# jolars/sgdnet

Measured on AMD Instinct MI355X. Metric: saga_epochs_per_sec, higher is better.
Workload: dtype f64

## Files before the change

sgdnet_amd/csrc/batched_geometry.hpp:

```cpp
#pragma once

#include <hip/hip_ext.h>

#include <type_traits>

#include "common.hpp"

#ifndef SGDNET_BIN_BLOCK
#define SGDNET_BIN_BLOCK 1024
#endif
#ifndef SGDNET_BIN_W
#define SGDNET_BIN_W 8
#endif
#ifndef SGDNET_RANGE_BLOCK
#define SGDNET_RANGE_BLOCK 512
#endif
#ifndef SGDNET_LDS_BLOCK
#define SGDNET_LDS_BLOCK 1024
#endif

namespace sgdnet {

constexpr int kGroup = 16;
constexpr int kBlock = 256;

constexpr int kD0Slots = 256;

constexpr int kCStride = 128;
constexpr uint32_t kIdMask = 0x1fffffffu;
constexpr int kInReg8 = 16;

constexpr int kLdsBlock = SGDNET_LDS_BLOCK;
constexpr int kDenseBlock = 256;
constexpr int kDenseVsBlock = 1024;
constexpr int kTileF = 64;

constexpr int kSlabElems = 32;
constexpr int kSlabGroups = kBlock / kSlabElems;

constexpr int kSyncLine = 32;
constexpr int kSyncGo = 0, kSyncExit = 1, kSyncStart = 2, kSyncCnt1 = 3, kSyncCnt2 = kSyncCnt1 + 8,
              kSyncXcd = kSyncCnt2 + 8;
constexpr int kFusedMaxBps = 128;
constexpr int kSyncLines = kSyncXcd + 8;
constexpr int kSyncSticky = kSyncLines;
constexpr int kSyncSeq = kSyncLines + 1;
constexpr int kFusedChunks = 3;
constexpr long long kFusedStartTicks = 2000000;
constexpr long long kFusedWaitTicks = 200000000;

struct __attribute__((aligned(16))) BinEntry {
  uint32_t t;
  uint32_t j;
  double x;
};
static_assert(sizeof(BinEntry) == 16, "bin entries are 16 bytes");

constexpr int kBinBlock = SGDNET_BIN_BLOCK;
constexpr int kBinDraws = kBinBlock / 2;
constexpr int kBinEntCap = 7 * kBinBlock;
constexpr int kBinW = SGDNET_BIN_W;
constexpr int kRangeBlock = SGDNET_RANGE_BLOCK;
constexpr size_t kRangeLdsBytes = 64 * 1024;

constexpr size_t kLdsPerCu = 160 * 1024;
constexpr size_t kLdsStaticReserve = 2 * 1024;
constexpr size_t kLdsTableMax = 80 * 1024;
constexpr int kLdsCap = 96 * 1024;
constexpr int kLdsAll = (int)(kLdsPerCu - kLdsStaticReserve);

template <typename F>
static int with_class_width(int kw, F&& f) {
  if (kw == 1) return f(std::integral_constant<int, 1>{});
  if (kw == 4) return f(std::integral_constant<int, 4>{});
  return f(std::integral_constant<int, 16>{});
}

static inline unsigned clamped_grid(int64_t work, int64_t per_block, int64_t most) {
  const int64_t grid = (work + per_block - 1) / per_block;
  return (unsigned)(grid < 1 ? 1 : grid > most ? most : grid);
// ... 31 lines not shown
```

sgdnet_amd/csrc/batched_plan.cpp:

```cpp
#include <mutex>
#include <set>
#include <utility>

#include "batched_geometry.hpp"
#include "r_rng_bodies.hpp"

namespace sgdnet {

int batched_max_classes() { return 64; }

int lds_target_grid(const SagaDev& d) {
  static const int forced = exp_env_int("SGDNET_LDS_GRID", 0);
  if (forced > 0) return forced;
  const int cus = d.cu_budget > 0 && d.cu_budget < 256 ? d.cu_budget : 256;
  const int g = cus - d.cu_reserve;
  return g < 64 ? 64 : g;
}

size_t binned_max_range_features(int K) { return kRangeLdsBytes / (sizeof(double) * (size_t)K); }

static size_t table_bytes(const SagaDev& d) { return sizeof(double) * (size_t)d.K * (size_t)d.p; }

int allow_dynamic_lds(const void* kernel, int bytes) {
  int dev = 0;
// ... 19 lines not shown
  if (!allow || d.K != 1 || d.Ky != 1 || d.xd || !d.ptr || d.p > 65536) return false;
  if (2 * sizeof(double) * (size_t)d.p + 16 + kLdsStaticReserve > (size_t)kLdsPerCu) return false;
  return (double)d.n * 2.0 * kCStride <= 48e9 && d.n < (int64_t)kIdMask;
}

int compact_entries(const SagaDev& d) { return d.family == SGDNET_BINOMIAL && d.y_binary ? 12 : 11; }

bool wants_binned(const SagaDev& d, int64_t batch) {
  static const int allow = exp_env_int("SGDNET_BINNED", 1);
  return allow && !d.xd && d.rec && d.idx && d.K <= 64 && !d.force_global && d.p < (1ll << 31) &&
         (d.K > 16 || (table_bytes(d) > kLdsTableMax && batch >= 4096));
}

bool wants_tiles(const SagaDev& d) { return d.xd && d.K <= 64 && (d.K > 16 || table_bytes(d) > kLdsTableMax); }

bool vs_eligible(const SagaDev& d) {
  if (d.V < 2 || d.K < 1 || d.K > 16 || (d.standardize && !(d.vcw && d.c)) || d.force_global || !d.vw) return false;
  const size_t table = table_bytes(d);
  if (d.xd) return table <= kLdsTableMax;
  if (d.K > 1) return d.rec && table <= kLdsTableMax;
  return 2 * table + 16 + kLdsStaticReserve <= kLdsPerCu;
}

static int vs_grid(const SagaDev& d) { return d.v_bps * d.V; }

static int64_t fused_slice(const SagaDev& d) { return 2 * ((d.p + 2 * (int64_t)d.v_bps - 1) / (2 * (int64_t)d.v_bps)); }
static size_t fused_lds_bytes(const SagaDev& d) {
  const int64_t part = (int64_t)(kLdsBlock / 64) * fused_slice(d);
  return sizeof(double) * (size_t)(d.p + (part > d.p ? part : d.p)) + 16;
}
size_t vs_fused_sync_words() { return (size_t)(kSyncLines + 2) * kSyncLine; }
size_t vs_fused_sync_sticky_word() { return (size_t)kSyncSticky * kSyncLine; }
size_t vs_fused_col_words() { return (size_t)kFusedMaxBps * kSyncLine; }
size_t vs_fused_exchange_doubles(const SagaDev& d, int n_shards) {
  return (size_t)n_shards * (size_t)(2 * d.p + 2) + (size_t)n_shards * kFusedMaxBps;
}
size_t vs_fused_publish_doubles(const SagaDev& d, int n_shards) { return (size_t)2 * n_shards * (size_t)(2 * d.p + 2); }

bool vs_fused_eligible(const SagaDev& d) {
  if (!vs_eligible(d) || d.K != 1 || d.xd || !d.cP || !lanes8_ok(d) || (d.p & 1) || !d.vsync || !d.vx || !d.vcol || !d.vpub) return false;
  if (d.v_bps < 1 || d.v_bps > kFusedMaxBps || d.V * d.v_bps > 1024) return false;
  if (fused_slice(d) > 2 * 64 * kFusedChunks) return false;
  if ((int64_t)d.V * d.v_bps * d.p * 8 >= (1ll << 31)) return false;
  return fused_lds_bytes(d) + kLdsStaticReserve <= kLdsPerCu;
}

static int vs_fused_rng_workgroups(const SagaDev& d) { return d.rngdev ? d.cu_reserve : 0; }

BatchPlan plan_batch(const SagaDev& d, int m, const PlanInputs& in) {
  BatchPlan g{};
  g.kw = class_width(d.K);
  const size_t table = table_bytes(d);
  if (d.V > 1 && vs_eligible(d)) {
    const int rng_wgs = vs_fused_rng_workgroups(d);
    g.slab_doubles = (int64_t)vs_grid(d) * d.K * d.p;
    if (in.fused && vs_fused_eligible(d) && vs_grid(d) + rng_wgs <= in.cus) {
      g.form = BatchForm::kFusedEpoch;
      g.grid = vs_grid(d) + rng_wgs;
      g.lds_bytes = fused_lds_bytes(d);
      if (rng_wgs > 0 && g.lds_bytes < kJumpLds) g.lds_bytes = kJumpLds;
      return g;
    }
    g.form = BatchForm::kShards;
    g.grid = vs_grid(d);
    int dpb = (m + d.v_bps - 1) / d.v_bps;
    g.lds_bytes = table;
// ... 87 lines not shown
```

sgdnet_amd/csrc/batched_shards.hip:

```cpp
#include "batched_k1.hpp"
#include "r_rng_bodies.hpp"

namespace sgdnet {

template <int KMAX>
__global__ __launch_bounds__(kBlock) void saga_vs_sweep_kernel(SagaDev d, LamParams* lamp, int tail, int nfb) {
  __shared__ double part[kSlabGroups][kSlabElems];
  __shared__ double red[kBlock / 64];
  __shared__ double sh_d0[KMAX];
  const SweepParams q = load_sweep_params(d, lamp, tail, SweepOverride{0.0, 0.0, 0.0});
  const int K = KMAX == 1 ? 1 : d.K;
  const int F = kSlabElems / K;
  const int E = F * K;
  const int v = (int)blockIdx.x / nfb, fb = (int)blockIdx.x - v * nfb;
  const int64_t KP = (int64_t)K * d.p;
  const double n_d = d.v_size[v];
  const int e = threadIdx.x % kSlabElems, g = threadIdx.x / kSlabElems;
  const int64_t elem = (int64_t)fb * E + e;
  const int64_t j_own = (int64_t)fb * F + threadIdx.x;
  const bool updates = (int)threadIdx.x < F && j_own < d.p;
  double w_old[KMAX], g_old[KMAX], c_own = 0.0;
#pragma unroll
  for (int k = 0; k < KMAX; ++k) {
    w_old[k] = g_old[k] = 0.0;
// ... 244 lines not shown
  __syncthreads();
  double t = 0.0;
#pragma unroll
  for (int wv = 0; wv < kLdsBlock / 64; ++wv) t += red[wv];
  __syncthreads();
  return t;
}

__device__ __forceinline__ void fused_leave(const SagaDev& d, LamParams* lamp, int nb, bool epoch_done) {
  asm volatile("s_waitcnt vmcnt(0)" ::: "memory");
  __syncthreads();
  if (threadIdx.x < 64) {
    unsigned* sync = d.vsync;
    unsigned prev = 0u;
    if (threadIdx.x == 0) {
      if (epoch_done && blockIdx.x == 0) {
        end_epoch(lamp, nb);
        if (d.n_peers > 1) __hip_atomic_fetch_add(sync + kSyncSeq * kSyncLine, 1u, __ATOMIC_RELAXED, __HIP_MEMORY_SCOPE_AGENT);
      }
      prev = __hip_atomic_fetch_add(sync + kSyncExit * kSyncLine, 1u, __ATOMIC_RELAXED, __HIP_MEMORY_SCOPE_AGENT);
    }
    prev = (unsigned)__shfl((int)prev, 0);
    if (prev + 1u == gridDim.x) {
      const int lane = (int)threadIdx.x;
      for (int wd = lane; wd < kSyncLines; wd += 64)
        __hip_atomic_store(sync + wd * kSyncLine, 0u, __ATOMIC_RELAXED, __HIP_MEMORY_SCOPE_AGENT);
      if (!(d.n_peers > 1))
        for (int wd = lane; wd < kFusedMaxBps; wd += 64)
          __hip_atomic_store(d.vcol + wd * kSyncLine, 0u, __ATOMIC_RELAXED, __HIP_MEMORY_SCOPE_AGENT);
      if (lane == 0 && d.rngdev && lamp->rng_generate) d.rngdev->gen += 1u;
    }
  }
}

template <bool kPeers>
__global__ __launch_bounds__(kLdsBlock) void saga_vs_epoch_kernel(SagaDev d, LamParams* lamp, int nb, int every) {
  extern __shared__ __attribute__((aligned(16))) double Dl[];
  __shared__ int ticket_counter;
  __shared__ int sh_ok;
  __shared__ double sh_red[kLdsBlock / 64];
  __shared__ double sh_val[4];
  const int tid = threadIdx.x;
  const int64_t p = d.p;
  const int64_t P2 = p >> 1;
  const int S = d.v_bps, V = d.V;
  if ((int)blockIdx.x >= V * S) {
    if (d.rngdev && lamp->rng_generate) {
      const RngDev* R = d.rngdev;
      const unsigned gen = R->gen;
      uint32_t* lds = reinterpret_cast<uint32_t*>(Dl);
      const int rb = (int)blockIdx.x - V * S, nrb = (int)gridDim.x - V * S;
      mt_state_body(rb, nrb, reinterpret_cast<uint32_t(*)[2][kMtN + 1]>(lds), R->state[gen & 1u], R->ends,
                    R->stream + (int64_t)(gen & 1u) * R->n, R->n, R->seg, R->gens);
      __syncthreads();
      mt_jump_body(rb, nrb, lds, R->state[gen & 1u], R->state[(gen + 1u) & 1u], R->poly, R->gens);
    }
    fused_leave(d, lamp, nb, false);
    return;
  }
  const int v = (int)blockIdx.x % V, wi = (int)blockIdx.x / V;
  const int F = 2 * (int)((p + 2 * S - 1) / (2 * S));
  const int j0 = wi * F;
  const int jn = p - j0 < F ? (p - j0 > 0 ? (int)(p - j0) : 0) : F;
  double* Wl = Dl + p;
  f64x2_t* D2 = reinterpret_cast<f64x2_t*>(Dl);
  f64x2_t* W2 = reinterpret_cast<f64x2_t*>(Wl);
// ... 15 lines not shown
      if (u < vv) lo += x;
      if (u == vv) own = x;
    }
    sh_par[6] = own;
    sh_par[7] = lo;
    sh_par[8] = tot;
  }
  const int64_t m_full = lamp->m_full;
  const int64_t sbase = lamp->stream_base;
  const bool raw_words = lamp->stream_raw != 0;
  const int64_t dps = d.v_dps;
  const bool std_x = d.standardize != 0;
  const int64_t L = 2 * p + 2;
  double* vwv = d.vw + (int64_t)v * p;
  double* vGv = d.vG + (int64_t)v * p;
  double* refv = d.vx + (int64_t)v * L;
  double* cwp = d.vx + (int64_t)V * L;
  unsigned* sync = d.vsync;
  const __amdgpu_buffer_rsrc_t rs_slab = fused_rsrc(d.slab, (int64_t)V * S * p * 8);
  const __amdgpu_buffer_rsrc_t rs_w = fused_rsrc(vwv, p * 8);
  const uint32_t* const stream_v = d.stream + sbase + (int64_t)v * dps;
  typedef K1CompactT<true> K1Epoch;
  const double* const draw_par = sh_par + 6;

#ifdef SGDNET_PHASE_TIMING
  unsigned long long ph_t = 0;
  if (d.dbg && tid == 0) d.dbg[(size_t)blockIdx.x * 16 + 14] = ph_t = phase_stamp();
#define FPH(slot)                                                 \
  do {                                                            \
    if (d.dbg && tid == 0) {                                      \
      const unsigned long long now = phase_stamp();               \
      d.dbg[(size_t)blockIdx.x * 16 + (slot)] += now - ph_t;      \
      d.dbg[(size_t)blockIdx.x * 16 + 15] = ph_t = now;           \
    }                                                             \
  } while (0)
#else
#define FPH(slot) ((void)0)
#endif
  if (tid == 0) {
    const unsigned xcc = __builtin_amdgcn_s_getreg((3 << 11) | 20) & 15u;
    __hip_atomic_fetch_or(sync + (kSyncXcd + v) * kSyncLine, 1u << xcc, __ATOMIC_RELAXED, __HIP_MEMORY_SCOPE_AGENT);
    asm volatile("s_waitcnt vmcnt(0)" ::: "memory");
    __hip_atomic_fetch_add(sync + kSyncStart * kSyncLine, 1u, __ATOMIC_RELAXED, __HIP_MEMORY_SCOPE_AGENT);
  }
  constexpr int kStage = 8;
  uint32_t s_first = 0u, s_second = 0u;
  {
    K1Epoch nx;
    nx.begin(d, stream_v, (int)(dps < m_full ? dps : m_full), wi, S, &ticket_counter);
    nx.raw = raw_words;
    nx.par = draw_par;
    f64x2_t t[kStage];
#pragma unroll
    for (int q = 0; q < kStage; ++q) {
      const int64_t i = tid + (int64_t)q * kLdsBlock;
      t[q] = f64x2_t{0.0, 0.0};
      if (i < P2) t[q] = reinterpret_cast<const f64x2_t*>(d.w)[i];
    }
    if (tid == 64) sh_val[2] = d.b[0];
    __syncthreads();
    nx.tag_first();
    s_first = nx.s_cur;
    s_second = nx.s_nxt;
    if (tid == 0) {
      sh_ok = fused_start(sync, lamp, (unsigned)(V * S)) ? 1 : 0;
      if (sh_ok) {
        const unsigned mask = sync_load(sync, kSyncXcd + v);
        sh_ok = (mask & (mask - 1u)) == 0u ? 3 : 1;
      }
    }
// ... 26 lines not shown
  int mi = 0;
  for (int r = 0; alive && r < nb; ++r) {
    const int64_t t0 = (int64_t)r * m_full;
    const int m = (int)(dps - t0 < m_full ? dps - t0 : m_full);
    const bool tail = m != m_full;
    const bool last = r + 1 == nb;
    const bool merge_due = last || (r + 1) % every == 0;

    if (tid == 0) ticket_counter = K1Epoch::static_tickets();
    K1Epoch cg;
    cg.init(d, stream_v + t0, m, wi, S, &ticket_counter);
    cg.raw = raw_words;
    cg.par = draw_par;
    cg.s_cur = s_first;
    cg.s_nxt = s_second;
    if (r > 0) cg.tag_first();
    int ts = threadIdx.x;
    asm volatile("" : "+v"(ts));
    double cw = 0.0, bv = 0.0;
    if ((ts >> 6) == 0) {
      if (std_x && r > 0)
        for (int k = ts & 63; k < S; k += 64) cw += ld_sc1(cwp + v * kFusedMaxBps + k);
      bv = r == 0 ? sh_val[2] : ld_sc1(d.vb + v);
    }
    if (r > 0) {
      for (int64_t i0 = ts; i0 < P2; i0 += (int64_t)kLdsBlock * kStage) {
        f64x2_t t[kStage];
#pragma unroll
        for (int q = 0; q < kStage; ++q) {
          const int64_t i = i0 + (int64_t)q * kLdsBlock;
          t[q] = f64x2_t{0.0, 0.0};
          if (i < P2) t[q] = ld2_sc1(rs_w, (uint32_t)(i * 16));
        }
#pragma unroll
        for (int q = 0; q < kStage; ++q) {
          const int64_t i = i0 + (int64_t)q * kLdsBlock;
          if (i < P2) W2[i] = t[q];
        }
      }
    }
    if ((ts >> 6) == 0) {
      cw = wave_sum(cw);
      if ((ts & 63) == 0) sh_val[0] = bv - cw;
    }
    __syncthreads();
    if (r == 0 && std_x) {
      double a = 0.0;
      for (int64_t j = ts; j < p; j += kLdsBlock) a += d.c[j] * Wl[j];
      a = fused_block_sum(a, sh_red);
      if (ts == 0) sh_val[0] -= a;
      __syncthreads();
    }
    const double b0 = sh_val[0];
    FPH(0);
#ifdef SGDNET_PHASE_TIMING
    if (d.dbg && tid == 0 && r == 0) d.dbg[(size_t)blockIdx.x * 16 + 8] = ph_t - ph_go;
#endif

    const double gct = cg.run(d, b0, Wl, Dl);
    __syncthreads();
    FPH(1);
    int tq = threadIdx.x;
    asm volatile("" : "+v"(tq));
    const int lane = tq & 63, wave = tq >> 6;
    const int64_t t0n = t0 + m_full;
    const int mn = (int)(dps - t0n < m_full ? dps - t0n : m_full);

    {
      const uint32_t base = (uint32_t)(((int64_t)blockIdx.x * p) * 8);
      for (int64_t i = tq; i < P2; i += kLdsBlock) {
        st2_shard(D2[i], rs_slab, base + (uint32_t)(i * 16), local);
        D2[i] = f64x2_t{0.0, 0.0};
      }
      const double t = wave_sum(gct);
      if (lane == 0) sh_red[wave] = t;
      __syncthreads();
      if (tq == 0) {
        double tot = 0.0;
        for (int wv = 0; wv < kLdsBlock / 64; ++wv) tot += sh_red[wv];
        st_shard(d.vd0 + blockIdx.x, tot, local);
      }
    }
    fused_arrive(sync, kSyncCnt1 + v);
    FPH(2);
    const bool upd = tq < jn;
    const bool icpt = wi == 0 && tq == jn;
    const bool act = upd || icpt;
    const int64_t j = j0 + tq;
    const int64_t oa = upd ? j : 2 * p, ob = upd ? p + j : 2 * p + 1;
    double* const rep_a = upd ? vGv + j : d.vgb + v;
    double* const rep_b = upd ? vwv + j : d.vb + v;
    const double* const own_a = upd ? d.G + j : d.gb;
    const double* const own_b = upd ? d.w + j : d.b;
    double a_old = 0.0, b_old = 0.0, c_own = 0.0, ra = 0.0, rb = 0.0;
    if (act) {
      a_old = r == 0 ? *own_a : ld_sc1(rep_a);
      b_old = r == 0 ? *own_b : ld_sc1(rep_b);
      if (std_x && upd) c_own = d.c[j];
      if (merge_due) {
        ra = mi == 0 ? *own_a : ld_sc1(refv + oa);
        rb = mi == 0 ? *own_b : ld_sc1(refv + ob);
      }
    }
    if (tq == 0) sh_ok = fused_poll(sync, kSyncCnt1 + v, (unsigned)S * (unsigned)(r + 1), lamp) ? 1 : 0;
    __syncthreads();
    if (!sh_ok) break;
    FPH(3);

    {
      double gsum = 0.0;
      if (wave == kLdsBlock / 64 - 1)
        for (int k = lane; k < S; k += 64) gsum += ld_sc1(d.vd0 + k * V + v);
      f64x2_t acc[kFusedChunks];
#pragma unroll
      for (int c = 0; c < kFusedChunks; ++c) acc[c] = f64x2_t{0.0, 0.0};
      for (int k = wave; k < S; k += 2 * (kLdsBlock / 64)) {
        const bool two = k + kLdsBlock / 64 < S;
        const uint32_t o0 = (uint32_t)((((int64_t)(k * V + v)) * p + j0) * 8);
        const uint32_t o1 = (uint32_t)((((int64_t)((k + kLdsBlock / 64) * V + v)) * p + j0) * 8);
        f64x2_t a0[kFusedChunks], a1[kFusedChunks];
#pragma unroll
        for (int c = 0; c < kFusedChunks; ++c) {
          const int pi = c * 64 + lane;
          a0[c] = a1[c] = f64x2_t{0.0, 0.0};
          if (2 * pi < jn) {
            a0[c] = ld2_sc1(rs_slab, o0 + (uint32_t)(pi * 16));
            if (two) a1[c] = ld2_sc1(rs_slab, o1 + (uint32_t)(pi * 16));
          }
        }
#pragma unroll
        for (int c = 0; c < kFusedChunks; ++c) {
          acc[c] += a0[c];
          acc[c] += a1[c];
        }
      }
#pragma unroll
      for (int c = 0; c < kFusedChunks; ++c) {
        const int pi = c * 64 + lane;
        if (2 * pi < F) reinterpret_cast<f64x2_t*>(Wl + (int64_t)wave * F)[pi] = acc[c];
      }
      if (wave == kLdsBlock / 64 - 1) {
        gsum = wave_sum(gsum);
        if (lane == 0) sh_val[1] = gsum;
      }
    }
    __syncthreads();
    double a_new = a_old, b_new = b_old;
    {
      const double d0 = sh_val[1];
      const double n_d = sh_par[6], gamma = sh_par[0];
      if (upd) {
        double dj = 0.0;
#pragma unroll
        for (int wv = 0; wv < kLdsBlock / 64; ++wv) dj += Wl[(int64_t)wv * F + tq];
        if (std_x) dj -= c_own * d0;
        const double beta = sh_par[1];
        const double r_m = tail ? sh_par[4] : sh_par[2], ls_m = tail ? sh_par[5] : sh_par[3];
        const double val = r_m * b_old - (gamma * ls_m) * a_old - gamma * dj;
        const double tau = beta * gamma * ls_m;
        b_new = val;
        if (penalty == SGDNET_ELASTICNET) {
          b_new = soft_threshold(val, tau);
        } else if (penalty == SGDNET_GROUPLASSO) {
          const double factor = tau / sqrt(val * val);
          b_new = factor < 1.0 ? val * (1.0 - factor) : 0.0;
        }
        a_new = (dj != 0.0 || penalty == SGDNET_GROUPLASSO) ? a_old + dj / n_d : a_old;
      } else if (icpt && d.fit_intercept) {
        const double dk = d0 / n_d;
        a_new = a_old + dk;
        b_new = b_old - gamma * (a_new * (d.xd ? 1.0 : 0.01) * (double)m + dk);
      }
    }
    FPH(4);
    if (merge_due) {
      const FusedPeers* PR = kPeers ? d.peers : nullptr;
      const int NP = kPeers ? d.n_peers : 1;
      double* pubv = d.vpub + (int64_t)((mi & 1) * V + v) * L;
      if (PR) {
        if (act) {
          st_sys(pubv + oa, a_new);
          st_sys(pubv + ob, b_new);
        }
        asm volatile("s_waitcnt vmcnt(0)" ::: "memory");
        __syncthreads();
        if (tq == 0)
          for (int q = 0; q < NP; ++q)
            __hip_atomic_fetch_add(PR->sync[q] + wi * kSyncLine, 1u, __ATOMIC_RELAXED, __HIP_MEMORY_SCOPE_SYSTEM);
      } else {
        if (act) {
          st_sc1(pubv + oa, a_new);
          st_sc1(pubv + ob, b_new);
        }
        fused_arrive(d.vcol, wi);
      }
      if (tq == 0)
        sh_ok = fused_poll(d.vcol, wi, (unsigned)(NP * V) * (col_base + (unsigned)(mi + 1)), lamp, PR != nullptr, sync) ? 1 : 0;
      __syncthreads();
      if (!sh_ok) break;
      double ma = ra, mb = rb;
      const double tot_all = PR ? PR->tot_size : sh_par[8];
      for (int q = 0; q < NP; ++q) {
        const double* pub0 = (PR ? PR->pub[q] : d.vpub) + (int64_t)((mi & 1) * V) * L;
        double xa[8], xb[8];
#pragma unroll
        for (int u = 0; u < 8; ++u) {
          xa[u] = xb[u] = 0.0;
          if (u < V && act) {
            xa[u] = PR ? ld_sys(pub0 + (int64_t)u * L + oa) : ld_sc1(pub0 + (int64_t)u * L + oa);
            xb[u] = PR ? ld_sys(pub0 + (int64_t)u * L + ob) : ld_sc1(pub0 + (int64_t)u * L + ob);
          }
        }
#pragma unroll
        for (int u = 0; u < 8; ++u) {
          if (u < V) {
            const double wt = (PR ? PR->vsize[q][u] : d.v_size[u]) / tot_all;
            ma += wt * (xa[u] - ra);
            mb += wt * (xb[u] - rb);
          }
        }
      }
      if (act) {
        a_new = ma;
        b_new = mb;
        if (!last || v == 0) {
          st_sc1(refv + oa, ma);
          st_sc1(refv + ob, mb);
        }
        if (last && v == 0) {
          *const_cast<double*>(own_a) = ma;
          *const_cast<double*>(own_b) = mb;
        }
      }
      ++mi;
      FPH(5);
    }
    if (act) {
      st_shard(rep_a, a_new, local);
      st_shard(rep_b, b_new, local);
    }
    if (std_x && !last) {
      const double a = fused_block_sum(upd ? c_own * b_new : 0.0, sh_red);
      if (tq == 0) st_shard(cwp + v * kFusedMaxBps + wi, a, local);
    }
    if (last) {
      done = true;
      break;
    }
    fused_arrive(sync, kSyncCnt2 + v);
    FPH(6);
    {
      K1Epoch nx;
      nx.begin(d, stream_v + t0n, mn, wi, S, &ticket_counter);
      s_first = nx.s_cur;
      s_second = nx.s_nxt;
    }
    if (tq == 0) sh_ok = fused_poll(sync, kSyncCnt2 + v, (unsigned)S * (unsigned)(r + 1), lamp) ? 1 : 0;
    __syncthreads();
    if (!sh_ok) break;
    FPH(7);
  }

#ifdef SGDNET_PHASE_TIMING
  if (d.dbg && tid == 0) ph_t = phase_stamp();
#endif
  fused_leave(d, lamp, nb, done);
#ifdef SGDNET_PHASE_TIMING
// ... 41 lines not shown
```

sgdnet_amd/csrc/common.hpp:

```cpp
#pragma once

#include <hip/hip_runtime.h>
#include <stdint.h>

#include "sgdnet_hip.h"

#ifdef SGDNET_EXPERIMENTS
#define SGD_ABLATE(d, bits) (((d).ablate & (bits)) != 0)
#else
#define SGD_ABLATE(d, bits) false
#endif

#include <stdlib.h>

namespace sgdnet {

void set_error(const char* fmt, ...);

#ifdef SGDNET_EXPERIMENTS
inline int exp_env_int(const char* name, int dflt) {
  const char* e = getenv(name);
  return e ? atoi(e) : dflt;
}
inline const char* exp_env_str(const char* name) { return getenv(name); }
// ... 203 lines not shown
struct PlanInputs {
  int64_t batch;
  bool bins_disabled;
  bool fused;
  int cus;
};
BatchPlan plan_batch(const SagaDev& d, int m, const PlanInputs& in);
bool wants_binned(const SagaDev& d, int64_t batch);
bool wants_tiles(const SagaDev& d);
bool vs_eligible(const SagaDev& d);
bool vs_fused_eligible(const SagaDev& d);
int launch_batch_gather(const SagaDev& d, const BatchPlan& g, LamParams* lam, int64_t t0_in_epoch, int m,
                        int batch_id_offset, hipStream_t st, hipEvent_t ev0 = nullptr, hipEvent_t ev1 = nullptr);
int launch_batch_sweep(const SagaDev& d, const BatchPlan& g, LamParams* lam, int penalty, int tail, int batch_id_offset,
                       hipStream_t st, hipEvent_t ev0 = nullptr, hipEvent_t ev1 = nullptr, double ov_r = 0.0,
                       double ov_ls = 0.0, double ov_m = 0.0);
int launch_vs_gather(const SagaDev& d, const BatchPlan& g, LamParams* lam, int64_t t0_in_epoch, int m, hipStream_t st,
                     hipEvent_t ev0 = nullptr, hipEvent_t ev1 = nullptr, int batch_index = 0);
int launch_vs_sweep(const SagaDev& d, const BatchPlan& g, LamParams* lam, int tail, hipStream_t st,
                    hipEvent_t ev0 = nullptr, hipEvent_t ev1 = nullptr);
int launch_vs_epoch(const SagaDev& d, const BatchPlan& g, LamParams* lam, int nb, int every, hipStream_t st,
                    hipEvent_t ev0 = nullptr, hipEvent_t ev1 = nullptr);
int allow_dynamic_lds(const void* kernel, int bytes);
template <typename F>
int allow_dynamic_lds(F* kernel, int bytes) { return allow_dynamic_lds(reinterpret_cast<const void*>(kernel), bytes); }
int launch_cw_init(const SagaDev& d, const LamParams* lam, hipStream_t st);
int launch_epoch_end(LamParams* lam, int batches, hipStream_t st);
int launch_vs_broadcast(const SagaDev& d, hipStream_t st);
int launch_vs_merge(const SagaDev& d, int final_merge, hipStream_t st, LamParams* epoch_end = nullptr, int batches = 0);
int launch_vs_cw(const SagaDev& d, hipStream_t st);
size_t vs_fused_sync_words();
size_t vs_fused_sync_sticky_word();
size_t vs_fused_col_words();
size_t vs_fused_publish_doubles(const SagaDev& d, int n_shards);
size_t vs_fused_exchange_doubles(const SagaDev& d, int n_shards);
bool compact_eligible(const SagaDev& d);
int launch_pack_compact(const SagaDev& d, char* P, char* Q, uint32_t* meta, hipStream_t st);
int compact_entries(const SagaDev& d);
int launch_m_move(const SagaDev& d, int to_record, hipStream_t st);

int launch_convergence(const SagaDev& d, LamParams* lam, hipStream_t st);
int launch_loss(const SagaDev& d, LamParams* lam, bool sparse, hipStream_t st);
int launch_delta_export(const SagaDev& d, const double* ref, double* out, double weight, hipStream_t st);
int launch_delta_apply(const SagaDev& d, double* ref, const double* merged, double w_weight, hipStream_t st);
int batched_max_classes();
int lds_target_grid(const SagaDev& d);
int launch_col_count(const SagaDev& d, int64_t nnz, unsigned* counts, hipStream_t st);
int launch_wpad_refresh(const SagaDev& d, hipStream_t st);
int launch_range_moment(const SagaDev& d, const uint16_t* feat_range, unsigned long long* sumsq, int R, hipStream_t st);
size_t binned_max_range_features(int K);
int launch_rng_fill(const uint32_t* state_in, uint32_t* state_out, uint32_t n_samples, uint32_t* out,
                    int64_t count, hipStream_t st, int n_shards = 0, const double* shard_size = nullptr,
                    int gens = 1, int64_t run_len = 0, int convert = 1, int narrow_cus = 0, int wgs = 0);
int launch_rng_convert(uint32_t* out, int64_t count, uint32_t n_samples, hipStream_t st, int n_shards,
                       const double* shard_size, int64_t run_len, int narrow_cus = 0);

bool mt_jump_poly(uint64_t J, uint32_t* out624);
void mt_jump_host(const sgdnet_rng* in, const uint32_t* poly624, sgdnet_rng* out);
int launch_rng_unif(const uint32_t* state_in, uint32_t* state_out, uint32_t* raw, double* out, int64_t count, hipStream_t st);
int launch_rng_jump(const uint32_t* state_in, uint32_t* state_out, const uint32_t* poly_dev, int gens,
                    hipStream_t st, int max_wgs = 0);
int rng_generators_per_workgroup();

}
```

sgdnet_amd/csrc/phase_report.cpp:

```cpp
#ifdef SGDNET_PHASE_TIMING
#include <stdio.h>
#include <stdlib.h>

#include <algorithm>
#include <vector>

#include "solver_state.hpp"

namespace sgdnet {

int phase_report_exact(const sgdnet_solver* s, const ExactPlan& plan, int epochs, int64_t draws_per_epoch) {
  if (plan.form == ExactForm::kDenseSmall2 && s->d.dbg && epochs > 0) {
    unsigned long long c[5];
    SGD_HIP_TRY(hipMemcpy(c, s->d.dbg + 24, sizeof(c), hipMemcpyDeviceToHost));
    (void)hipMemset(s->d.dbg + 24, 0, sizeof(c));
    const double its = (double)epochs * (double)draws_per_epoch;
    fprintf(stderr, "[sgdnet] small dense kernel with feeder, consumer cycles per draw: slot+history %.0f, dot %.0f, gradient+store %.0f, "
                    "intercept %.0f, step+penalty+average %.0f\n", c[0] / its, c[1] / its, c[2] / its, c[3] / its, c[4] / its);
  }
  if (plan.form == ExactForm::kSparseK1m && s->d.dbg && epochs > 0) {
    (void)hipDeviceSynchronize();
    unsigned long long c[5];
    SGD_HIP_TRY(hipMemcpy(c, s->d.dbg + 16, sizeof(c), hipMemcpyDeviceToHost));
    (void)hipMemset(s->d.dbg + 16, 0, sizeof(c));
// ... 17 lines not shown
    (void)hipMemset(s->d.dbg, 0, sizeof(ph));
    const double its = (double)epochs * (double)draws_per_epoch;
    fprintf(stderr, "[sgdnet] wide exact kernel, cycles per iteration (thread 0): loads+dot+sum %.0f, scale %.0f, barrier A %.0f, "
                    "class %.0f, barrier B %.0f, step %.0f\n",
            (double)ph[0] / its, (double)ph[1] / its, (double)ph[2] / its, (double)ph[3] / its, (double)ph[4] / its, (double)ph[5] / its);
  }
  return SGDNET_OK;
}

int phase_report_batched(const sgdnet_solver* s, int64_t batch, bool fused_prof) {
  if (s->d.dbg && fused_prof) {
    const int grid = s->d.V * s->d.v_bps;
    std::vector<unsigned long long> t(16 * 1024);
    SGD_HIP_TRY(hipMemcpy(t.data(), s->d.dbg, sizeof(unsigned long long) * t.size(), hipMemcpyDeviceToHost));
    static const char* nm[8] = {"stage w + ids", "draw loop", "publish slab", "wait shard (1)", "slice sweep", "merge",
                                "store + arrive", "wait shard (2)"};
    unsigned long long first = ~0ull, last = 0;
    for (int b = 0; b < grid; ++b) {
      first = std::min(first, t[b * 16 + 14]);
      last = std::max(last, t[b * 16 + 15]);
    }
    fprintf(stderr, "[phase] fused epoch kernel: span seen by the workgroups %.1f us (%d workgroups)\n", (double)(last - first) / 100.0, grid);
    double tot_mean = 0;
    for (int ph = 0; ph < 8; ++ph) {
      double sum = 0, mx = 0, mn = 1e30;
      for (int b = 0; b < grid; ++b) {
        const double dt = (double)t[b * 16 + ph] / 100.0;
        sum += dt; mx = std::max(mx, dt); mn = std::min(mn, dt);
      }
      tot_mean += sum / grid;
      fprintf(stderr, "[phase] %-16s per epoch: mean %7.1f us  min %7.1f  max %7.1f\n", nm[ph], sum / grid, mn, mx);
    }
    fprintf(stderr, "[phase] sum of the means %.1f us\n", tot_mean);
    static const char* bn[3] = {"entry -> go seen", "go -> draw loop 0", "last stores -> out"};
    const int bs[3] = {10, 8, 9};
    for (int k = 0; k < 3; ++k) {
      double sum = 0, mx = 0, mn = 1e30;
      for (int b = 0; b < grid; ++b) {
        const double dt = (double)t[b * 16 + bs[k]] / 100.0;
        sum += dt; mx = std::max(mx, dt); mn = std::min(mn, dt);
      }
      fprintf(stderr, "[phase] %-18s per launch: mean %6.1f us  min %6.1f  max %6.1f\n", bn[k], sum / grid, mn, mx);
    }
    for (int v = 0; v < s->d.V; ++v) {
      double a0 = 0, a1 = 0;
      for (int b = v * s->d.v_bps; b < (v + 1) * s->d.v_bps; ++b) {
        a0 += (double)(t[b * 16 + 14] - first) / 100.0;
        a1 += (double)(t[b * 16 + 15] - first) / 100.0;
      }
      fprintf(stderr, "[phase]   shard %d: mean start %.1f us, mean end %.1f us\n", v, a0 / s->d.v_bps, a1 / s->d.v_bps);
    }
  } else
  if (s->d.dbg && plan(s, batch, batch).form == BatchForm::kBinned) {
    std::vector<unsigned long long> t(16 * 1024);
    SGD_HIP_TRY(hipMemcpy(t.data(), s->d.dbg, sizeof(unsigned long long) * t.size(), hipMemcpyDeviceToHost));
    static const char* nm[10] = {"gather: init", "gather: draw loop", "gather: barrier", "gather: reserve runs",
                                 "gather: place entries", "", "sweep: zero + first entries", "sweep: entries -> LDS",
                                 "sweep: barrier", "sweep: update features"};
    for (int ph = 0; ph < 10; ++ph) {
      if (ph == 5) continue;
      double sum = 0, mx = 0;
      int cnt = 0;
      for (int b = 0; b < 1024; ++b) {
        if (!t[b * 16 + ph] || !t[b * 16 + ph + 1] || t[b * 16 + ph + 1] < t[b * 16 + ph]) continue;
        const double dt = (double)(t[b * 16 + ph + 1] - t[b * 16 + ph]) / 100.0;
        sum += dt; mx = std::max(mx, dt); ++cnt;
// ... 66 lines not shown
```

sgdnet_amd/csrc/solver_epoch.cpp:

```cpp
#include <math.h>
#include <stdlib.h>
#include <stdio.h>
#include <string.h>

#include <algorithm>
#include <chrono>
#include <vector>

#include "solver_state.hpp"

namespace sgdnet {

static bool lam_on_device(const sgdnet_solver* s) {
  if (!s->lam_dev_valid) return false;
  const LamParams &a = s->lam, &b = s->lam_dev_mirror;
  return a.penalty == b.penalty && a.gamma == b.gamma && a.alpha == b.alpha && a.beta == b.beta && a.r_full == b.r_full &&
         a.ls_full == b.ls_full && a.r_tail == b.r_tail && a.ls_tail == b.ls_tail && a.m_full == b.m_full &&
         a.m_tail == b.m_tail && a.stream_base == b.stream_base && a.stream_wrap == b.stream_wrap &&
         a.draws_per_epoch == b.draws_per_epoch && a.batch_seq == b.batch_seq && a.stream_raw == b.stream_raw &&
         a.rng_generate == b.rng_generate;
}

static void lam_advance(sgdnet_solver* s, int64_t draws, int batches) {
  for (LamParams* q : {&s->lam, &s->lam_dev_mirror}) {
// ... 578 lines not shown
      bool rerun = false;
      (void)fused_recover(s, 2, 0, 0, &rerun);
      drop_graph(s);
      set_error("batched mode: a fused epoch launch %s; the epochs enqueued since the last synchronisation are void "
                "(sgdnet_set_option(\"fused_epoch\", 0) keeps the separate launches)",
                code == 1 ? "could not become resident on the GPU (is it shared with another process?)"
                          : "timed out inside the epoch");
      return SGDNET_EHIP;
    }
  }
  SGD_HIP_TRY(hipStreamSynchronize(s->st));
  return check_bins(s);
}

int sgdnet_solver_profile_epoch(sgdnet_solver* s, int64_t batch, int64_t stream_offset,
                                int64_t draws_per_epoch, double* gather_ms, int* gather_launches,
                                double* sweep_ms, int* sweep_launches) {
  if (!s || draws_per_epoch <= 0 || !s->penalty_set) {
    set_error("sgdnet_solver_profile_epoch: invalid argument");
    return SGDNET_EINVAL;
  }
  SGD_HIP_TRY(hipSetDevice(s->device));
  int rc = begin_batched_epochs(s, batch, stream_offset, draws_per_epoch, draws_per_epoch, 1, &batch);
  if (rc) return rc;
  struct Events {
    std::vector<hipEvent_t> v;
    ~Events() {
      for (hipEvent_t e : v) (void)hipEventDestroy(e);
    }
  } events;
  std::vector<hipEvent_t>& ev = events.v;
#ifdef SGDNET_PHASE_TIMING
  const bool fused_prof = fused_epochs(s);
  if (fused_prof && s->d.dbg) SGD_HIP_TRY(hipMemsetAsync(s->d.dbg, 0, sizeof(unsigned long long) * 16 * 1024, s->st));
#endif
  rc = enqueue_epoch_kernels(s, batch, draws_per_epoch, &ev);
  if (rc) return rc;
  SGD_HIP_TRY(hipStreamSynchronize(s->st));
  lam_advance(s, draws_per_epoch, n_batches(batch, draws_per_epoch));
  double g = 0.0, w = 0.0;
  int ng = 0;
  for (size_t i = 0; i + 3 < ev.size(); i += 4) {
    float ms = 0.f;
    SGD_HIP_TRY(hipEventElapsedTime(&ms, ev[i], ev[i + 1]));
    g += ms;
    SGD_HIP_TRY(hipEventElapsedTime(&ms, ev[i + 2], ev[i + 3]));
    w += ms;
    ++ng;
  }
#ifdef SGDNET_PHASE_TIMING
  rc = phase_report_batched(s, batch, fused_prof);
  if (rc) return rc;
#endif
  if (gather_ms) *gather_ms = g;
  if (gather_launches) *gather_launches = ng;
  if (sweep_ms) *sweep_ms = w;
  if (sweep_launches) *sweep_launches = ng;
  return SGDNET_OK;
}

int sgdnet_solver_gather_form(const sgdnet_solver* s, int64_t batch) {
  if (!s || batch < 1) return 0;
  const BatchPlan g = plan(s, batch, batch);
  if (g.form == BatchForm::kFusedEpoch) return 3;
  if (g.form == BatchForm::kBinned) return 2;
  if (g.form == BatchForm::kShards) {
    SagaDev d = s->d;
// ... 125 lines not shown
```

sgdnet_amd/csrc/solver_shards.cpp:

```cpp
#include <string.h>

#include <hip/hip_ext.h>

#include "solver_state.hpp"

using namespace sgdnet;

static void free_virtual_shards(sgdnet_solver* s) {
  for (void* q : s->vs_owned) (void)hipFree(q);
  s->vs_owned.clear();
  SagaDev& d = s->d;
  d.V = 0;
  d.vw = d.vG = d.vb = d.vgb = d.vd0 = d.vref = d.vcw = d.vx = d.vpub = nullptr;
  d.vsync = d.vcol = nullptr;
  d.peers = nullptr;
  d.n_peers = 0;
}

extern "C" {

int sgdnet_solver_set_virtual_shards(sgdnet_solver* s, int n_shards) {
  if (!s || n_shards < 0 || n_shards > 8) {
    set_error("sgdnet_solver_set_virtual_shards: 0..8 shards");
    return SGDNET_EINVAL;
  }
  SGD_HIP_TRY(hipSetDevice(s->device));
  SGD_HIP_TRY(hipStreamSynchronize(s->st));
  drop_graph(s);
  free_virtual_shards(s);
  SagaDev& d = s->d;
  if (n_shards < 2) return SGDNET_OK;
  if (d.K > 16) {
    set_error("virtual shards: up to 16 classes");
    return SGDNET_EUNSUPPORTED;
  }
  const int64_t KP = (int64_t)d.K * d.p;
  auto alloc = [&](double** out, size_t count) -> int {
    void* q = nullptr;
    if (hipMalloc(&q, sizeof(double) * count) != hipSuccess) return SGDNET_ENOMEM;
    (void)hipMemset(q, 0, sizeof(double) * count);
    s->vs_owned.push_back(q);
    *out = static_cast<double*>(q);
    return SGDNET_OK;
  };
  int rc = alloc(&d.vw, (size_t)n_shards * KP);
  if (!rc) rc = alloc(&d.vG, (size_t)n_shards * KP);
  if (!rc) rc = alloc(&d.vb, 8 * (size_t)d.K);
  if (!rc) rc = alloc(&d.vgb, 8 * (size_t)d.K);
  if (!rc) rc = alloc(&d.vcw, 8 * (size_t)d.K);
  if (!rc) rc = alloc(&d.vd0, 256 * (size_t)d.K);
  if (!rc) rc = alloc(&d.vref, (size_t)(2 * KP + 2 * d.K));
  if (!rc && d.K == 1) {
    auto alloc_fg = [&](void** out, size_t bytes) -> int {
      void* q = nullptr;
      if (hipExtMallocWithFlags(&q, bytes, hipDeviceMallocFinegrained) != hipSuccess) {
        (void)hipGetLastError();
        if (hipMalloc(&q, bytes) != hipSuccess) return SGDNET_ENOMEM;
      }
      (void)hipMemset(q, 0, bytes);
      s->vs_owned.push_back(q);
      *out = q;
      return SGDNET_OK;
    };
    double* words = nullptr;
    rc = alloc(&words, (vs_fused_sync_words() * sizeof(unsigned) + sizeof(double) - 1) / sizeof(double));
    d.vsync = reinterpret_cast<unsigned*>(words);
    if (!rc) rc = alloc(&d.vx, vs_fused_exchange_doubles(d, n_shards));
    if (!rc) rc = alloc_fg(reinterpret_cast<void**>(&d.vcol), vs_fused_col_words() * sizeof(unsigned));
    if (!rc) rc = alloc_fg(reinterpret_cast<void**>(&d.vpub), vs_fused_publish_doubles(d, n_shards) * sizeof(double));
  }
  if (rc) {
    set_error("virtual shards: out of device memory");
    return rc;
  }
  d.V = n_shards;
  d.v_bps = lds_target_grid(d) / n_shards;
  const int64_t base = d.n / n_shards, rem = d.n % n_shards;
  for (int v = 0; v < 8; ++v) d.v_size[v] = v < n_shards ? (double)(base + (v < rem ? 1 : 0)) : 0.0;
  if (!vs_eligible(d)) {
    free_virtual_shards(s);
    set_error("virtual shards: n_features too large for the LDS-resident gather");
    return SGDNET_EUNSUPPORTED;
  }
// ... 182 lines not shown
```

Measured before the change: 1301.

## Publish per-wave d0 partials and split slab sweep across chunk-group wavefronts

```diff
diff --git a/sgdnet_amd/csrc/batched_geometry.hpp b/sgdnet_amd/csrc/batched_geometry.hpp
--- a/sgdnet_amd/csrc/batched_geometry.hpp
+++ b/sgdnet_amd/csrc/batched_geometry.hpp
@@ -46,6 +46,8 @@
 constexpr int kSyncSticky = kSyncLines;
 constexpr int kSyncSeq = kSyncLines + 1;
 constexpr int kFusedChunks = 3;
+constexpr int kFusedWaves = kLdsBlock / 64;
+constexpr int kFusedGroups = 5;
 constexpr long long kFusedStartTicks = 2000000;
 constexpr long long kFusedWaitTicks = 200000000;
 
diff --git a/sgdnet_amd/csrc/batched_plan.cpp b/sgdnet_amd/csrc/batched_plan.cpp
--- a/sgdnet_amd/csrc/batched_plan.cpp
+++ b/sgdnet_amd/csrc/batched_plan.cpp
@@ -75,6 +75,7 @@
 size_t vs_fused_sync_words() { return (size_t)(kSyncLines + 2) * kSyncLine; }
 size_t vs_fused_sync_sticky_word() { return (size_t)kSyncSticky * kSyncLine; }
 size_t vs_fused_col_words() { return (size_t)kFusedMaxBps * kSyncLine; }
+size_t vs_fused_d0_doubles() { return (size_t)1024 * kFusedWaves; }
 size_t vs_fused_exchange_doubles(const SagaDev& d, int n_shards) {
   return (size_t)n_shards * (size_t)(2 * d.p + 2) + (size_t)n_shards * kFusedMaxBps;
 }
diff --git a/sgdnet_amd/csrc/batched_shards.hip b/sgdnet_amd/csrc/batched_shards.hip
--- a/sgdnet_amd/csrc/batched_shards.hip
+++ b/sgdnet_amd/csrc/batched_shards.hip
@@ -300,6 +300,14 @@
     }
   }
 }
+
+#ifdef SGDNET_PHASE_TIMING
+__device__ __forceinline__ unsigned long long phase_stamp_issue() {
+  unsigned long long t;
+  asm volatile("s_memrealtime %0\n\ts_waitcnt lgkmcnt(0)" : "=s"(t)::"memory");
+  return t;
+}
+#endif
 
 template <bool kPeers>
 __global__ __launch_bounds__(kLdsBlock) void saga_vs_epoch_kernel(SagaDev d, LamParams* lamp, int nb, int every) {
@@ -381,10 +389,21 @@
       const unsigned long long now = phase_stamp();               \
       d.dbg[(size_t)blockIdx.x * 16 + (slot)] += now - ph_t;      \
       d.dbg[(size_t)blockIdx.x * 16 + 15] = ph_t = now;           \
+      ph_s = now;                                                 \
     }                                                             \
+  } while (0)
+  unsigned long long ph_s = ph_t;
+#define FSUB(sub, drain)                                                          \
+  do {                                                                            \
+    if (d.dbg && tid == 0) {                                                      \
+      const unsigned long long now = (drain) ? phase_stamp() : phase_stamp_issue(); \
+      d.dbg[(size_t)16 * 1024 + (size_t)blockIdx.x * 16 + (sub)] += now - ph_s;  \
+      ph_s = now;                                                                 \
+    }                                                                             \
   } while (0)
 #else
 #define FPH(slot) ((void)0)
+#define FSUB(sub, drain) ((void)0)
 #endif
   if (tid == 0) {
     const unsigned xcc = __builtin_amdgcn_s_getreg((3 << 11) | 20) & 15u;
@@ -477,6 +496,7 @@
           t[q] = f64x2_t{0.0, 0.0};
           if (i < P2) t[q] = ld2_sc1(rs_w, (uint32_t)(i * 16));
         }
+        FSUB(5, true);
 #pragma unroll
         for (int q = 0; q < kStage; ++q) {
           const int64_t i = i0 + (int64_t)q * kLdsBlock;
@@ -497,6 +517,7 @@
       __syncthreads();
     }
     const double b0 = sh_val[0];
+    FSUB(6, true);
     FPH(0);
 #ifdef SGDNET_PHASE_TIMING
     if (d.dbg && tid == 0 && r == 0) d.dbg[(size_t)blockIdx.x * 16 + 8] = ph_t - ph_go;
@@ -517,16 +538,12 @@
         st2_shard(D2[i], rs_slab, base + (uint32_t)(i * 16), local);
         D2[i] = f64x2_t{0.0, 0.0};
       }
+      FSUB(0, false);
       const double t = wave_sum(gct);
-      if (lane == 0) sh_red[wave] = t;
-      __syncthreads();
-      if (tq == 0) {
-        double tot = 0.0;
-        for (int wv = 0; wv < kLdsBlock / 64; ++wv) tot += sh_red[wv];
-        st_shard(d.vd0 + blockIdx.x, tot, local);
-      }
+      if (lane == 0) st_shard(d.vd0 + (int64_t)blockIdx.x * kFusedWaves + wave, t, local);
     }
     fused_arrive(sync, kSyncCnt1 + v);
+    FSUB(1, true);
     FPH(2);
     const bool upd = tq < jn;
     const bool icpt = wi == 0 && tq == jn;
@@ -553,40 +570,44 @@
     FPH(3);
 
     {
-      double gsum = 0.0;
-      if (wave == kLdsBlock / 64 - 1)
-        for (int k = lane; k < S; k += 64) gsum += ld_sc1(d.vd0 + k * V + v);
-      f64x2_t acc[kFusedChunks];
-#pragma unroll
-      for (int c = 0; c < kFusedChunks; ++c) acc[c] = f64x2_t{0.0, 0.0};
-      for (int k = wave; k < S; k += 2 * (kLdsBlock / 64)) {
-        const bool two = k + kLdsBlock / 64 < S;
-        const uint32_t o0 = (uint32_t)((((int64_t)(k * V + v)) * p + j0) * 8);
-        const uint32_t o1 = (uint32_t)((((int64_t)((k + kLdsBlock / 64) * V + v)) * p + j0) * 8);
-        f64x2_t a0[kFusedChunks], a1[kFusedChunks];
-#pragma unroll
-        for (int c = 0; c < kFusedChunks; ++c) {
-          const int pi = c * 64 + lane;
-          a0[c] = a1[c] = f64x2_t{0.0, 0.0};
-          if (2 * pi < jn) {
-            a0[c] = ld2_sc1(rs_slab, o0 + (uint32_t)(pi * 16));
-            if (two) a1[c] = ld2_sc1(rs_slab, o1 + (uint32_t)(pi * 16));
+      static_assert(kFusedChunks * kFusedGroups < kFusedWaves, "a wavefront per (chunk, group) and one for the sum of gc");
+      if (wave == kFusedWaves - 1) {
+        constexpr int kU = 8;
+        const int np = S * kFusedWaves;
+        double gsum = 0.0;
+        for (int i0 = lane; i0 < np; i0 += 64 * kU) {
+          double x[kU];
+#pragma unroll
+          for (int q = 0; q < kU; ++q) {
+            const int i = i0 + q * 64;
+            x[q] = 0.0;
+            if (i < np) x[q] = ld_sc1(d.vd0 + ((int64_t)(i / kFusedWaves) * V + v) * kFusedWaves + i % kFusedWaves);
           }
-        }
-#pragma unroll
-        for (int c = 0; c < kFusedChunks; ++c) {
-          acc[c] += a0[c];
-          acc[c] += a1[c];
-        }
-      }
-#pragma unroll
-      for (int c = 0; c < kFusedChunks; ++c) {
-        const int pi = c * 64 + lane;
-        if (2 * pi < F) reinterpret_cast<f64x2_t*>(Wl + (int64_t)wave * F)[pi] = acc[c];
-      }
-      if (wave == kLdsBlock / 64 - 1) {
+#pragma unroll
+          for (int q = 0; q < kU; ++q) gsum += x[q];
+        }
         gsum = wave_sum(gsum);
         if (lane == 0) sh_val[1] = gsum;
+      } else if (wave < kFusedChunks * kFusedGroups) {
+        constexpr int kU = 7;
+        const int c = wave / kFusedGroups, g = wave - c * kFusedGroups;
+        const int pi = c * 64 + lane;
+        f64x2_t acc = f64x2_t{0.0, 0.0};
+        if (2 * pi < jn) {
+          for (int k0 = g; k0 < S; k0 += kFusedGroups * kU) {
+            f64x2_t a[kU];
+#pragma unroll
+            for (int q = 0; q < kU; ++q) {
+              const int k = k0 + q * kFusedGroups;
+              a[q] = f64x2_t{0.0, 0.0};
+              if (k < S) a[q] = ld2_sc1(rs_slab, (uint32_t)((((int64_t)(k * V + v)) * p + j0) * 8) + (uint32_t)(pi * 16));
+            }
+#pragma unroll
+            for (int q = 0; q < kU; ++q) acc += a[q];
+          }
+        }
+        FSUB(2, true);
+        if (2 * pi < F) reinterpret_cast<f64x2_t*>(Wl + (int64_t)g * F)[pi] = acc;
       }
     }
     __syncthreads();
@@ -597,7 +618,8 @@
       if (upd) {
         double dj = 0.0;
 #pragma unroll
-        for (int wv = 0; wv < kLdsBlock / 64; ++wv) dj += Wl[(int64_t)wv * F + tq];
+        for (int g = 0; g < kFusedGroups; ++g) dj += Wl[(int64_t)g * F + tq];
+        FSUB(3, true);
         if (std_x) dj -= c_own * d0;
         const double beta = sh_par[1];
         const double r_m = tail ? sh_par[4] : sh_par[2], ls_m = tail ? sh_par[5] : sh_par[3];
@@ -617,6 +639,7 @@
         b_new = b_old - gamma * (a_new * (d.xd ? 1.0 : 0.01) * (double)m + dk);
       }
     }
+    FSUB(4, true);
     FPH(4);
     if (merge_due) {
       const FusedPeers* PR = kPeers ? d.peers : nullptr;
@@ -639,10 +662,12 @@
         }
         fused_arrive(d.vcol, wi);
       }
+      FSUB(7, true);
       if (tq == 0)
         sh_ok = fused_poll(d.vcol, wi, (unsigned)(NP * V) * (col_base + (unsigned)(mi + 1)), lamp, PR != nullptr, sync) ? 1 : 0;
       __syncthreads();
       if (!sh_ok) break;
+      FSUB(8, true);
       double ma = ra, mb = rb;
       const double tot_all = PR ? PR->tot_size : sh_par[8];
       for (int q = 0; q < NP; ++q) {
@@ -665,6 +690,7 @@
           }
         }
       }
+      FSUB(9, true);
       if (act) {
         a_new = ma;
         b_new = mb;
@@ -678,6 +704,7 @@
         }
       }
       ++mi;
+      FSUB(10, false);
       FPH(5);
     }
     if (act) {
diff --git a/sgdnet_amd/csrc/common.hpp b/sgdnet_amd/csrc/common.hpp
--- a/sgdnet_amd/csrc/common.hpp
+++ b/sgdnet_amd/csrc/common.hpp
@@ -259,6 +259,7 @@
 size_t vs_fused_sync_words();
 size_t vs_fused_sync_sticky_word();
 size_t vs_fused_col_words();
+size_t vs_fused_d0_doubles();
 size_t vs_fused_publish_doubles(const SagaDev& d, int n_shards);
 size_t vs_fused_exchange_doubles(const SagaDev& d, int n_shards);
 bool compact_eligible(const SagaDev& d);
diff --git a/sgdnet_amd/csrc/phase_report.cpp b/sgdnet_amd/csrc/phase_report.cpp
--- a/sgdnet_amd/csrc/phase_report.cpp
+++ b/sgdnet_amd/csrc/phase_report.cpp
@@ -73,6 +73,22 @@
       fprintf(stderr, "[phase] %-16s per epoch: mean %7.1f us  min %7.1f  max %7.1f\n", nm[ph], sum / grid, mn, mx);
     }
     fprintf(stderr, "[phase] sum of the means %.1f us\n", tot_mean);
+    {
+      std::vector<unsigned long long> u(16 * 1024);
+      SGD_HIP_TRY(hipMemcpy(u.data(), s->d.dbg + 16 * 1024, sizeof(unsigned long long) * u.size(), hipMemcpyDeviceToHost));
+      static const char* sn[11] = {"publish: stores issued", "publish: drained + arrived", "sweep: slab loads returned",
+                                   "sweep: LDS reduce", "sweep: update", "stage: loads returned", "stage: LDS written",
+                                   "merge: publish + arrive", "merge: poll", "merge: exchange loads", "merge: stores"};
+      const int order[11] = {5, 6, 0, 1, 2, 3, 4, 7, 8, 9, 10};
+      for (int k : order) {
+        double sum = 0, mx = 0, mn = 1e30;
+        for (int b = 0; b < grid; ++b) {
+          const double dt = (double)u[b * 16 + k] / 100.0;
+          sum += dt; mx = std::max(mx, dt); mn = std::min(mn, dt);
+        }
+        fprintf(stderr, "[phase]   %-26s per epoch: mean %6.1f us  min %6.1f  max %6.1f\n", sn[k], sum / grid, mn, mx);
+      }
+    }
     static const char* bn[3] = {"entry -> go seen", "go -> draw loop 0", "last stores -> out"};
     const int bs[3] = {10, 8, 9};
     for (int k = 0; k < 3; ++k) {
diff --git a/sgdnet_amd/csrc/solver_epoch.cpp b/sgdnet_amd/csrc/solver_epoch.cpp
--- a/sgdnet_amd/csrc/solver_epoch.cpp
+++ b/sgdnet_amd/csrc/solver_epoch.cpp
@@ -634,7 +634,7 @@
   std::vector<hipEvent_t>& ev = events.v;
 #ifdef SGDNET_PHASE_TIMING
   const bool fused_prof = fused_epochs(s);
-  if (fused_prof && s->d.dbg) SGD_HIP_TRY(hipMemsetAsync(s->d.dbg, 0, sizeof(unsigned long long) * 16 * 1024, s->st));
+  if (fused_prof && s->d.dbg) SGD_HIP_TRY(hipMemsetAsync(s->d.dbg, 0, sizeof(unsigned long long) * 16 * 2048, s->st));
 #endif
   rc = enqueue_epoch_kernels(s, batch, draws_per_epoch, &ev);
   if (rc) return rc;
diff --git a/sgdnet_amd/csrc/solver_shards.cpp b/sgdnet_amd/csrc/solver_shards.cpp
--- a/sgdnet_amd/csrc/solver_shards.cpp
+++ b/sgdnet_amd/csrc/solver_shards.cpp
@@ -48,7 +48,7 @@
   if (!rc) rc = alloc(&d.vb, 8 * (size_t)d.K);
   if (!rc) rc = alloc(&d.vgb, 8 * (size_t)d.K);
   if (!rc) rc = alloc(&d.vcw, 8 * (size_t)d.K);
-  if (!rc) rc = alloc(&d.vd0, 256 * (size_t)d.K);
+  if (!rc) rc = alloc(&d.vd0, d.K == 1 ? vs_fused_d0_doubles() : 256 * (size_t)d.K);
   if (!rc) rc = alloc(&d.vref, (size_t)(2 * KP + 2 * d.K));
   if (!rc && d.K == 1) {
     auto alloc_fg = [&](void** out, size_t bytes) -> int {
```

Result: no change. 1308, median of 5 (+0.6%).
